# merbanan/rtl_433

Hardware: NVIDIA H100
Metric: IQ MS/s end-to-end demod+slice (higher is better)
Workload: dtype u8/int16/int32 fixed point

## Files before the change

### rtl_433_b200/csrc/r433b_api.cu

```cuda
#include <algorithm>
#include <cmath>
#include <cstdio>
#include <cstdlib>
#include <chrono>
#include <cstring>
#include <exception>
#include <atomic>
#include <mutex>
#include <string>
#include <thread>
#include <vector>

#include "../../include/r433b.h"
#include "../../include/r433b_abi.h"
#include "r433b_kernels.cuh"
#include "r433b_host.hpp"
#include "r433b_pulses.hpp"
#include "r433b_analyze.cuh"
#include "r433b_analyze_host.hpp"
#include "r433b_grab.cuh"

using namespace r433b;

#ifdef R433B_SIMT_EMU
// ... 32 lines not shown
    r433b_batch batch{};
    std::vector<uint64_t> offsets, lengths;
    bool processed = false, fetched = false;
    unsigned fpdm = 0;
    int enable_fm = 0;
    int n_sms = 132;
    int spoil_front = 0;
    size_t min_caps[3] = {0, 0, 0};
    Levels lv{};
    DevBuf d_data, d_offsets, d_train, d_pkgs, d_ppool, d_gpool, d_counters, d_am, d_fm;
    DevBuf d_devparams, d_lists, d_pairs, d_arena, d_cursor;
    size_t pkg_cap = 0, pool_cap = 0, arena_cap = 0;
    unsigned n_ook = 0, n_fsk = 0;
    unsigned n_pkgs = 0, pool_used = 0;
    unsigned long long event_bytes = 0, n_events = 0, n_samples = 0, n_gated = 0;
    HostBuf h_pkgs, h_ppool, h_gpool, h_pairs, h_events;
    r433b_timing timing{};
    cudaEvent_t ev[6]{};
    int pipeline_groups = 0;
    cudaStream_t s_in = nullptr, s_det = nullptr, s_out = nullptr;
    static constexpr int kMaxGroups = 16;
    cudaEvent_t ev_in[kMaxGroups]{}, ev_det[kMaxGroups]{}, ev_slc[kMaxGroups]{}, ev_t[4 * kMaxGroups]{}, ev_f[kMaxGroups]{}, ev_init = nullptr;
    DevBuf d_order;
    DevBuf d_ranges, d_state, d_lengths, d_stage, d_raw, d_log, d_amoff, d_chunks, d_tiles;
    std::vector<uint64_t> am_offsets;
    HostBuf h_ranges;
    bool d2h_done = false;
    bool pulse_mode = false;
    std::vector<PulseSet::Meta> pulse_meta;
    std::vector<uint32_t> dev_index;
    bool analyzed = false;
    std::vector<r433b_analysis> an;
    std::vector<r433b_guess> an_guess;
    std::vector<std::string> an_text;
    std::vector<r433b_pair> an_pairs;
    std::vector<uint8_t> an_events;
    DevBuf d_an, d_an_dev, d_an_gap, d_an_pairs, d_an_arena;
    std::thread worker;
    bool in_flight = false;
    int worker_rc = 0;
    r433b_batch sub_batch{};
    std::vector<uint64_t> sub_offsets, sub_lengths;
    r433b_results sub_res{};
    uint8_t const *grab_src = nullptr;
    unsigned grab_flip = 0;
    std::vector<uint32_t> p_events;
// ... 144 lines not shown
    if (char const *v = getenv("R433B_TEST_CAPS")) {
        unsigned long long c[3] = {0, 0, 0};
        sscanf(v, "%llu,%llu,%llu", &c[0], &c[1], &c[2]);
        for (int i = 0; i < 3; ++i) ctx->min_caps[i] = (size_t)c[i];
    }
    if (cudaDeviceGetAttribute(&ctx->n_sms, cudaDevAttrMultiProcessorCount, cuda_device) != cudaSuccess || ctx->n_sms <= 0)
        ctx->n_sms = 132;
    *out = ctx;
    return R433B_OK;
}

void r433b_destroy(r433b_ctx *ctx)
{
    if (!ctx) return;
    if (ctx->worker.joinable()) ctx->worker.join();
    cudaSetDevice(ctx->device);
    for (r433b_chain *ch : ctx->chains) {
        chain_free_device(ch);
        ch->ctx = nullptr;
    }
    for (DevBuf *b : {&ctx->d_data, &ctx->d_offsets, &ctx->d_train, &ctx->d_pkgs, &ctx->d_ppool, &ctx->d_gpool,
                 &ctx->d_counters, &ctx->d_am, &ctx->d_fm, &ctx->d_devparams, &ctx->d_lists, &ctx->d_pairs,
                 &ctx->d_arena, &ctx->d_cursor, &ctx->d_ranges, &ctx->d_state, &ctx->d_lengths, &ctx->d_stage, &ctx->d_raw, &ctx->d_log, &ctx->d_amoff, &ctx->d_chunks, &ctx->d_tiles,
                 &ctx->d_order, &ctx->d_an, &ctx->d_an_dev, &ctx->d_an_gap, &ctx->d_an_pairs, &ctx->d_an_arena,
                 &ctx->d_grab_prior, &ctx->d_grab_segs, &ctx->d_grab_stage})
        if (b->p) cudaFree(b->p);
    for (HostBuf *b : {&ctx->h_pkgs, &ctx->h_ppool, &ctx->h_gpool, &ctx->h_pairs, &ctx->h_events, &ctx->h_ranges})
        if (b->p) cudaFreeHost(b->p);
    for (auto &v : ctx->ev)
        if (v) cudaEventDestroy(v);
    for (auto *arr : {ctx->ev_in, ctx->ev_det, ctx->ev_slc})
        for (int i = 0; i < r433b_ctx::kMaxGroups; ++i)
            if (arr[i]) cudaEventDestroy(arr[i]);
    for (auto &v : ctx->ev_t)
        if (v) cudaEventDestroy(v);
    for (auto &v : ctx->ev_f)
        if (v) cudaEventDestroy(v);
    if (ctx->ev_init) cudaEventDestroy(ctx->ev_init);
    for (cudaStream_t st : {ctx->s_in, ctx->s_det, ctx->s_out})
        if (st) cudaStreamDestroy(st);
    delete ctx;
}

char const *r433b_last_error(r433b_ctx const *ctx) { return ctx ? ctx->err.c_str() : "no context"; }

int r433b_set_levels(r433b_ctx *ctx, int use_mag_est, float level_limit_db, float min_level_db, float min_snr_db)
{
// ... 65 lines not shown

int upload_slicer_tables(r433b_ctx *ctx, std::vector<uint32_t> const &rates, cudaStream_t st)
{
    size_t const n_devs = ctx->devs.size();
    std::vector<SlicerParams> sp(rates.size() * n_devs);
    for (size_t g = 0; g < rates.size(); ++g)
        for (size_t i = 0; i < n_devs; ++i) {
            sp[g * n_devs + i] = scale_device(ctx->devs[i], rates[g]);
            if (!ctx->gates.empty()) sp[g * n_devs + i].gate = ctx->gates[i].min_bits;
        }
    std::vector<unsigned> lists = slice_list(ctx->devs, 1), fsk = slice_list(ctx->devs, 2);
    ctx->n_ook = (unsigned)lists.size();
    ctx->n_fsk = (unsigned)fsk.size();
    lists.insert(lists.end(), fsk.begin(), fsk.end());
    if (int r = dev_reserve(ctx, ctx->d_devparams, std::max<size_t>(1, sp.size()) * sizeof(SlicerParams))) return r;
    if (int r = dev_reserve(ctx, ctx->d_lists, (lists.size() + 1) * sizeof(unsigned))) return r;
    size_t const stage_threads = (size_t)ctx->n_sms * kSliceCtasPerSm * kSliceThreads;
    if (int r = dev_reserve(ctx, ctx->d_stage, stage_threads * kStageWords * sizeof(uint32_t))) return r;
    if (!sp.empty()) CU(cudaMemcpyAsync(ctx->d_devparams.p, sp.data(), sp.size() * sizeof(SlicerParams), cudaMemcpyHostToDevice, st));
    if (!lists.empty()) CU(cudaMemcpyAsync(ctx->d_lists.p, lists.data(), lists.size() * sizeof(unsigned), cudaMemcpyHostToDevice, st));
    return R433B_OK;
}

void launch_slice(r433b_ctx *ctx, GroupRange *range, unsigned n_pkgs, unsigned rate_index, cudaStream_t st)
{
    unsigned const n_devs = (unsigned)ctx->devs.size();
    r433b_package *pkgs = (r433b_package *)ctx->d_pkgs.p;
    SliceParams q{};
    q.pkgs = pkgs;
    q.range = range;
    q.order = (unsigned const *)ctx->d_order.p;
    q.pulse_pool = (int const *)ctx->d_ppool.p;
    q.gap_pool = (int const *)ctx->d_gpool.p;
    q.dev = (SlicerParams const *)ctx->d_devparams.p + (size_t)rate_index * n_devs;
    q.n_devs = n_devs;
    q.ook_list = (unsigned const *)ctx->d_lists.p;
    q.fsk_list = q.ook_list + ctx->n_ook;
    q.n_ook = ctx->n_ook;
    q.n_fsk = ctx->n_fsk;
    q.pairs = (r433b_pair *)ctx->d_pairs.p;
    q.arena = (uint8_t *)ctx->d_arena.p;
    q.arena_cap = ctx->arena_cap;
    q.cursor = (unsigned long long *)ctx->d_cursor.p;
    q.stage = (uint32_t *)ctx->d_stage.p;
    unsigned const bgrid = (unsigned)ctx->n_sms * 2;
    R4_LAUNCH(k_bucket_count, bgrid, kBucketThreads, 0, st, range, pkgs, n_pkgs, n_devs);
    R4_LAUNCH(k_bucket_scan, 1, 1, 0, st, range);
    R4_LAUNCH(k_bucket_scatter, bgrid, kBucketThreads, 0, st, range, (r433b_package const *)pkgs, n_pkgs, (unsigned *)ctx->d_order.p);
    R4_LAUNCH(k_slice2, (unsigned)ctx->n_sms * kSliceCtasPerSm, kSliceThreads, 0, st, q);
}

int slice_ranges(r433b_ctx *ctx, std::vector<GroupRange> const &ranges, unsigned n_pkgs, cudaStream_t st)
{
    unsigned const n_devs = (unsigned)ctx->devs.size();
    unsigned long long cursor[4] = {0, 0, 0, 0};
    ctx->timing.slice_launches = 0;
    CU(cudaEventRecord(ctx->ev[2], st));
    if (n_pkgs && n_devs) {
        size_t const pair_bytes = (size_t)n_pkgs * n_devs * sizeof(r433b_pair);
        if (int r = dev_reserve(ctx, ctx->d_pairs, pair_bytes)) return r;
        if (int r = dev_reserve(ctx, ctx->d_order, (size_t)n_pkgs * sizeof(unsigned))) return r;
        if (int r = dev_reserve(ctx, ctx->d_ranges, ranges.size() * sizeof(GroupRange))) return r;
        if (int r = dev_reserve(ctx, ctx->d_cursor, 64)) return r;
        for (int attempt = 0; attempt < 3; ++attempt) {
            if (int r = dev_reserve(ctx, ctx->d_arena, ctx->arena_cap)) return r;
            CU(cudaMemsetAsync(ctx->d_pairs.p, 0, pair_bytes, st));
            CU(cudaMemsetAsync(ctx->d_cursor.p, 0, 64, st));
            CU(cudaMemcpyAsync(ctx->d_ranges.p, ranges.data(), ranges.size() * sizeof(GroupRange), cudaMemcpyHostToDevice, st));
            for (size_t g = 0; g < ranges.size(); ++g) {
                launch_slice(ctx, (GroupRange *)ctx->d_ranges.p + g, n_pkgs, (unsigned)g, st);
                CU(cudaGetLastError());
                ctx->timing.slice_launches++;
            }
            CU(cudaMemcpyAsync(cursor, ctx->d_cursor.p, sizeof(cursor), cudaMemcpyDeviceToHost, st));
            CU(cudaStreamSynchronize(st));
            if (!cursor[2]) break;
            ctx->arena_cap = (size_t)cursor[0] + (1u << 20);
            if (attempt == 2) return fail(ctx, R433B_EOVERFLOW, "event arena overflow");
        }
    }
    CU(cudaEventRecord(ctx->ev[3], st));
    CU(cudaEventSynchronize(ctx->ev[3]));
    cudaEventElapsedTime(&ctx->timing.slice_ms, ctx->ev[2], ctx->ev[3]);
    ctx->event_bytes = cursor[0];
// ... 235 lines not shown
        if (ctx->offsets[i + 1] - ctx->offsets[i] != stride) uniform = false;
    if (G == 0) {
        uint64_t const min_slice = SS == 4 ? (512u << 10) : (128u << 10);
        G = (total_bytes >= (256ull << 20) && stride >= (1u << 20)) ? (int)std::min<uint64_t>(r433b_ctx::kMaxGroups, stride / min_slice) : 1;
    }
    if (b->data_on_device && ctx->pipeline_groups == 0) G = 1;
    if (b->want_stages || !n_devs || !uniform || cf32) G = 1;
    uint64_t slice_samples = 0;
    if (G > 1) {
        uint64_t n_samp = stride / SS;
        uint64_t unit = (uint64_t)T;
        slice_samples = (n_samp / G + unit - 1) / unit * unit;
        if (slice_samples == 0 || slice_samples >= n_samp) G = 1;
        else G = (int)((n_samp + slice_samples - 1) / slice_samples);
        if (G > r433b_ctx::kMaxGroups) G = 1;
    }
    if (G > 1) {
        using clk = std::chrono::steady_clock;
        auto t_wall0 = clk::now();
        if (int r = dev_reserve(ctx, ctx->d_pkgs, ctx->pkg_cap * sizeof(r433b_package))) return r;
        if (int r = dev_reserve(ctx, ctx->d_order, ctx->pkg_cap * sizeof(unsigned))) return r;
        if (int r = dev_reserve(ctx, ctx->d_ppool, ctx->pool_cap * sizeof(int))) return r;
        if (int r = dev_reserve(ctx, ctx->d_gpool, ctx->pool_cap * sizeof(int))) return r;
        size_t const pair_cap_bytes = ctx->pkg_cap * n_devs * sizeof(r433b_pair);
        if (int r = dev_reserve(ctx, ctx->d_pairs, pair_cap_bytes)) return r;
        if (int r = dev_reserve(ctx, ctx->d_arena, ctx->arena_cap)) return r;
        if (int r = dev_reserve(ctx, ctx->d_ranges, G * sizeof(GroupRange))) return r;
        if (int r = dev_reserve(ctx, ctx->d_state, (size_t)b->n_streams * sizeof(StreamState))) return r;
        if (int r = host_reserve(ctx, ctx->h_ranges, G * sizeof(GroupRange))) return r;
        dp.pkgs = (r433b_package *)ctx->d_pkgs.p;
        dp.pkg_cap = (unsigned)std::min<size_t>(ctx->pkg_cap, 0xffffffffu);
        dp.pulse_pool = (int *)ctx->d_ppool.p;
        dp.gap_pool = (int *)ctx->d_gpool.p;
        dp.pool_cap = (unsigned)std::min<size_t>(ctx->pool_cap, 0xffffffffu);
        if (!ch) dp.state = (StreamState *)ctx->d_state.p;
        detect_ran = true;
        GroupRange *d_rg = (GroupRange *)ctx->d_ranges.p;
        GroupRange *h_rg = (GroupRange *)ctx->h_ranges.p;
        unsigned const *d_cnt = (unsigned const *)ctx->d_counters.p;
        unsigned long long const *d_cur = (unsigned long long const *)ctx->d_cursor.p;

        CU(cudaEventRecord(ctx->ev_init, 0));
        CU(cudaStreamWaitEvent(ctx->s_det, ctx->ev_init, 0));
        CU(cudaMemsetAsync(ctx->d_counters.p, 0, 64, ctx->s_det));
        CU(cudaMemsetAsync(ctx->d_cursor.p, 0, 64, ctx->s_det));
        CU(cudaMemsetAsync(ctx->d_pairs.p, 0, pair_cap_bytes, ctx->s_det));
// ... 127 lines not shown
        dp.pulse_pool = (int *)ctx->d_ppool.p;
        dp.gap_pool = (int *)ctx->d_gpool.p;
        dp.pool_cap = (unsigned)std::min<size_t>(ctx->pool_cap, 0xffffffffu);
        CU(cudaMemsetAsync(ctx->d_counters.p, 0, 64, st));
        if (b->n_streams) {
            launch_detect(dp, st, ctx->ev[4]);
            CU(cudaGetLastError());
            detect_launches++;
            detect_ran = true;
        }
        CU(cudaMemcpyAsync(counters, ctx->d_counters.p, sizeof(counters), cudaMemcpyDeviceToHost, st));
        CU(cudaStreamSynchronize(st));
        if (!counters[2]) break;
        ctx->pkg_cap = std::max<size_t>(ctx->pkg_cap, (size_t)counters[0] + 64);
        ctx->pool_cap = std::max<size_t>(ctx->pool_cap, (size_t)counters[1] + 4096);
        if (attempt == 2) return fail(ctx, R433B_EOVERFLOW, "package arena overflow");
    }
    if ((uint64_t)counters[0] * n_devs > 0xffffffffull)
        return fail(ctx, R433B_EOVERFLOW, "packages x devices exceeds the 32-bit pair index (r433b_package.first_pair)");
    ctx->n_pkgs = counters[0];
    ctx->pool_used = counters[1];
    GroupRange all{};
    all.pkg_end = ctx->n_pkgs;
    if (int r = slice_ranges(ctx, std::vector<GroupRange>{all}, ctx->n_pkgs, st)) return r;
    ctx->n_samples = used_bytes / SS;
    cudaEventElapsedTime(&ctx->timing.h2d_ms, ctx->ev[0], ctx->ev[1]);
    ctx->timing.front_ms = 0;
    if (detect_launches) {
        cudaEventElapsedTime(&ctx->timing.front_ms, ctx->ev[1], ctx->ev[4]);
        cudaEventElapsedTime(&ctx->timing.detect_ms, ctx->ev[4], ctx->ev[2]);
    } else
        cudaEventElapsedTime(&ctx->timing.detect_ms, ctx->ev[1], ctx->ev[2]);
    ctx->timing.front_launches = detect_launches;
    ctx->timing.front_redone = counters[4];
    ctx->timing.front_repairs = counters[5];
    ctx->timing.idle_skipped = counters[6];
    ctx->timing.idle_rewalks = counters[7];
    ctx->timing.chain_folds = counters[8];
    ctx->timing.chain_fm_rebuilds = counters[9];
    cudaEventElapsedTime(&ctx->timing.total_ms, ctx->ev[0], ctx->ev[3]);
    ctx->timing.d2h_ms = 0;
    ctx->timing.detect_launches = detect_launches;
    ctx->processed = true;
    finish_chain();
    return R433B_OK;
}

// ... 501 lines not shown
        ranges.back().pkg_end = j + 1;
    }
    for (uint32_t rate : rates)
        if (!rate) return fail(ctx, R433B_EINVAL, "a package has sample_rate 0");

    ctx->n_pkgs = n;
    ctx->pool_used = (unsigned)pp.size();
    ctx->n_samples = 0;
    ctx->event_bytes = ctx->n_events = ctx->n_gated = 0;
    ctx->timing = r433b_timing{};
    if (n) {
        if (int r = dev_reserve(ctx, ctx->d_pkgs, (size_t)n * sizeof(r433b_package))) return r;
        if (int r = dev_reserve(ctx, ctx->d_ppool, pp.size() * sizeof(int) + 16)) return r;
        if (int r = dev_reserve(ctx, ctx->d_gpool, gp.size() * sizeof(int) + 16)) return r;
        CU(cudaMemcpyAsync(ctx->d_pkgs.p, hp.data(), (size_t)n * sizeof(r433b_package), cudaMemcpyHostToDevice, st));
        CU(cudaMemcpyAsync(ctx->d_ppool.p, pp.data(), pp.size() * sizeof(int), cudaMemcpyHostToDevice, st));
        CU(cudaMemcpyAsync(ctx->d_gpool.p, gp.data(), gp.size() * sizeof(int), cudaMemcpyHostToDevice, st));
        CU(cudaStreamSynchronize(st));
    }
    if (n && n_devs) {
        size_t const arena_min = ctx->min_caps[2] ? ctx->min_caps[2] : (size_t)(1u << 20);
        if (ctx->arena_cap < arena_min) ctx->arena_cap = arena_min;
        if (int r = upload_slicer_tables(ctx, rates, st)) return r;
        if (int r = slice_ranges(ctx, ranges, n, st)) return r;
        ctx->timing.total_ms = ctx->timing.slice_ms;
    }
    ctx->processed = true;
    return R433B_OK;
}

}



namespace {

uint32_t package_rate(r433b_ctx const *ctx, r433b_package const &k)
{
    if (ctx->pulse_mode && k.end_pos < ctx->pulse_meta.size()) return ctx->pulse_meta[k.end_pos].rate;
    return ctx->batch.samp_rate;
}

}

extern "C" {

int r433b_analyze(r433b_ctx *ctx, r433b_results const *res)
// ... 389 lines not shown
```

### rtl_433_b200/csrc/r433b_kernels.cuh

```cuda
#pragma once
#include <cuda_runtime.h>
#include <stdint.h>

#include "../../include/r433b.h"
#include "r433b_core.cuh"
#include "r433b_slice.cuh"
#include "r433b_detect.cuh"

namespace r433b {


__global__ void k_cf32_to_cs16(float4 const *in, uint2 *out, size_t n4)
{
    for (size_t i = (size_t)blockIdx.x * blockDim.x + threadIdx.x; i < n4; i += (size_t)gridDim.x * blockDim.x) {
        float4 v = __ldcs(in + i);
        float f[4] = {v.x, v.y, v.z, v.w};
        int s[4];
#pragma unroll
        for (int k = 0; k < 4; ++k) {
            float t = __fmul_rn(f[k], 32767.0f);
            int q = (t >= -2147483648.0f && t < 2147483648.0f) ? __float2int_rz(t) : (int)0x80000000;
            q = q < -32767 ? -32767 : (q > 32767 ? 32767 : q);
            s[k] = q;
        }
        uint2 o;
        o.x = (uint32_t)(uint16_t)(int16_t)s[0] | ((uint32_t)(uint16_t)(int16_t)s[1] << 16);
        o.y = (uint32_t)(uint16_t)(int16_t)s[2] | ((uint32_t)(uint16_t)(int16_t)s[3] << 16);
        out[i] = o;
    }
}


constexpr int kLenBuckets = 4;
__host__ __device__ inline int len_bucket(unsigned num_pulses)
{
    return num_pulses < 64 ? 0 : num_pulses < 160 ? 1 : num_pulses < 400 ? 2 : 3;
}

struct GroupRange {
    unsigned pkg_begin, pkg_end;
    unsigned pool_begin, pool_end;
    unsigned long long arena_begin, arena_end;
    unsigned long long events_end, gated_end;
    unsigned overflow;
    unsigned next;
    unsigned seg_begin[2][kLenBuckets], seg_count[2][kLenBuckets], seg_fill[2][kLenBuckets];
    unsigned groups[2];
};

__global__ void k_mark(GroupRange *r, int which, unsigned const *counters, unsigned long long const *cursor)
{
    if (which == 0) {
        r->pkg_begin = counters[0];
        r->pool_begin = counters[1];
    } else if (which == 1) {
        r->pkg_end = counters[0];
        r->pool_end = counters[1];
        r->overflow = counters[2];
        r->next = 0;
        for (int i = 0; i < 2 * kLenBuckets; ++i) (&r->seg_count[0][0])[i] = 0;
    } else if (which == 2) {
        r->arena_begin = cursor[0];
    } else {
        r->arena_end = cursor[0];
        r->events_end = cursor[1];
        r->gated_end = cursor[3];
        r->overflow |= (unsigned)cursor[2] << 1;
    }
}


constexpr int kBucketThreads = 256;
__global__ void __launch_bounds__(kBucketThreads) k_bucket_count(GroupRange *r, r433b_package *pkgs, unsigned n_pkgs, unsigned n_devs)
{
    unsigned const b0 = r->pkg_begin, b1 = r->pkg_end < n_pkgs ? r->pkg_end : n_pkgs;
    for (unsigned pk = b0 + blockIdx.x * kBucketThreads + threadIdx.x; pk < b1; pk += gridDim.x * kBucketThreads) {
        r433b_package const k = pkgs[pk];
        pkgs[pk].first_pair = pk * n_devs;
        atomicAdd(&r->seg_count[k.type == 1 ? 0 : 1][len_bucket(k.num_pulses)], 1u);
    }
}

__global__ void k_bucket_scan(GroupRange *r)
{
    unsigned at = 0;
    for (int t = 0; t < 2; ++t) {
        unsigned g = 0;
        for (int b = 0; b < kLenBuckets; ++b) {
            r->seg_begin[t][b] = at;
            r->seg_fill[t][b] = 0;
            at += r->seg_count[t][b];
            g += (r->seg_count[t][b] + 31) / 32;
        }
        r->groups[t] = g;
    }
    r->next = 0;
}

__global__ void __launch_bounds__(kBucketThreads) k_bucket_scatter(GroupRange *r, r433b_package const *pkgs, unsigned n_pkgs, unsigned *order)
{
    unsigned const b0 = r->pkg_begin, b1 = r->pkg_end < n_pkgs ? r->pkg_end : n_pkgs;
    for (unsigned pk = b0 + blockIdx.x * kBucketThreads + threadIdx.x; pk < b1; pk += gridDim.x * kBucketThreads) {
        r433b_package const k = pkgs[pk];
        int const t = k.type == 1 ? 0 : 1, b = len_bucket(k.num_pulses);
        unsigned const pos = r->seg_begin[t][b] + atomicAdd(&r->seg_fill[t][b], 1u);
        order[b0 + pos] = pk;
    }
}

struct SliceParams {
    r433b_package const *pkgs;
    GroupRange *range;
    unsigned const *order;
    int const *pulse_pool, *gap_pool;
    SlicerParams const *dev;
    unsigned n_devs;
    unsigned const *ook_list, *fsk_list;
    unsigned n_ook, n_fsk;
    r433b_pair *pairs;
    uint8_t *arena;
    unsigned long long arena_cap;
    unsigned long long *cursor;
    uint32_t *stage;
};

constexpr int kSliceThreads = 128;
constexpr unsigned kStageWords = 1024;
constexpr int kSliceCtasPerSm = 8;

__shared__ uint32_t g_slice_win[kSliceWindow][kSliceThreads];
__shared__ unsigned g_slice_seg[2][kSliceThreads];
struct SliceWindow {
    static constexpr bool kOn = true;
    __device__ __forceinline__ static uint32_t &slot(unsigned s) { return g_slice_win[s][threadIdx.x]; }
};

__global__ void __launch_bounds__(kSliceThreads, kSliceCtasPerSm) k_slice2(SliceParams p)
{
    unsigned const lane = threadIdx.x & 31, warp = threadIdx.x >> 5;
    GroupRange const *rg = p.range;
    unsigned const pk_begin = rg->pkg_begin;
    unsigned const groups_ook = rg->groups[0], groups_fsk = rg->groups[1];
    unsigned const items_ook = p.n_ook * groups_ook, items = items_ook + p.n_fsk * groups_fsk;
    uint32_t *stage = p.stage + ((size_t)blockIdx.x * kSliceThreads + threadIdx.x) * kStageWords;
    for (;;) {
        unsigned item = 0;
        if (lane == 0) item = atomicAdd(&p.range->next, 1u);
        item = __shfl_sync(0xffffffffu, item, 0);
        if (item >= items) break;
        int const t = item < items_ook ? 0 : 1;
        unsigned const rel = t ? item - items_ook : item;
        unsigned const groups = t ? groups_fsk : groups_ook;
        unsigned const slot = rel / groups;
        unsigned g = rel - slot * groups;
        unsigned const dev = (t ? p.fsk_list : p.ook_list)[slot];
        int b = 0;
        for (; b < kLenBuckets - 1; ++b) {
            unsigned const gb = (rg->seg_count[t][b] + 31) / 32;
            if (g < gb) break;
            g -= gb;
        }
        unsigned const in_seg = g * 32 + lane;
        bool const active = in_seg < rg->seg_count[t][b];
        unsigned const pk = active ? p.order[pk_begin + rg->seg_begin[t][b] + in_seg] : 0;
        SlicerParams const sp = p.dev[dev];
        PulseView pv;
        pv.pulse = p.pulse_pool;
        pv.gap = p.gap_pool;
        pv.n = 0;
        if (active) {
            r433b_package const k = p.pkgs[pk];
            pv.pulse = p.pulse_pool + k.pulse_off;
            pv.gap = p.gap_pool + k.pulse_off;
            pv.n = k.num_pulses;
        }
        unsigned bytes = 0, nev = 0, ng1 = 0, ngN = 0, wb = 0;
        if (active) {
            EventWriterT<SliceWindow> w;
            w.init(stage, kStageWords, (unsigned)sp.gate);
            slice_dispatch(pv, sp, w);
            bytes = w.committed * 4;
            wb = w.wb;
            nev = w.events;
            ng1 = w.gated1;
            ngN = w.gatedN;
        }
        unsigned incl = bytes;
#pragma unroll
        for (int o = 1; o < 32; o <<= 1) {
            unsigned v = __shfl_up_sync(0xffffffffu, incl, o);
            if ((int)lane >= o) incl += v;
        }
        unsigned const total = __shfl_sync(0xffffffffu, incl, 31);
        unsigned evs = nev, dropped = ng1 + ngN;
#pragma unroll
        for (int o = 16; o > 0; o >>= 1) {
            evs += __shfl_xor_sync(0xffffffffu, evs, o);
            dropped += __shfl_xor_sync(0xffffffffu, dropped, o);
// ... 54 lines not shown
```

### rtl_433_b200/csrc/r433b_slice.cuh

```cuda
#pragma once
#include <stdint.h>
#include "r433b_core.cuh"

namespace r433b {

constexpr int kBbRows = 50;
constexpr int kBbCols = 128;

#ifdef __CUDA_ARCH__
R4_HD float fmul(float a, float b) { return __fmul_rn(a, b); }
R4_HD float fadd(float a, float b) { return __fadd_rn(a, b); }
R4_HD float fdiv(float a, float b) { return __fdiv_rn(a, b); }
R4_HD double dadd(double a, double b) { return __dadd_rn(a, b); }
R4_HD double dmul(double a, double b) { return __dmul_rn(a, b); }
#else
R4_HD float fmul(float a, float b) { volatile float r = a * b; return r; }
R4_HD float fadd(float a, float b) { volatile float r = a + b; return r; }
R4_HD float fdiv(float a, float b) { volatile float r = a / b; return r; }
R4_HD double dadd(double a, double b) { volatile double r = a + b; return r; }
R4_HD double dmul(double a, double b) { volatile double r = a * b; return r; }
#endif

struct SlicerParams {
    int modulation;
// ... 231 lines not shown
        } else if ((bits > max_bits ? bits : max_bits) < gate) {
            if (num_rows == 1) gated1++; else gatedN++;
            reset_event();
            return;
        } else if (one_word) {
            pos = ev_start + 1;
        } else {
            close_row();
            if (dirty) {
                put(pos, row_hw);
                pos += 1;
            }
        }
        put(ev_start, one_word ? 0xffu | (bits << 8) | (syncs << 13) | (bswap32(acc) << 16)
                               : num_rows | (dirty ? 0x80u : 0u) | (free_row << 8) | ((pos - ev_start) << 16));
        committed = pos;
        events++;
        reset_event();
    }
};
using EventWriter = EventWriterT<>;


struct PulseView {
    int const *pulse;
    int const *gap;
    unsigned n;
};

enum {
    kModOokMc = 3, kModOokPcm = 4, kModOokPpm = 5, kModOokPwm = 6, kModOokPiwmRaw = 8, kModOokDmc = 9,
    kModOokOsv1 = 10, kModOokPiwmDc = 11, kModOokNrzs = 12, kModOokRzi = 13,
    kModFskPcm = 16, kModFskPwm = 17, kModFskMc = 18
};

R4_HD bool device_takes(int modulation, int package_type)
{
    if (package_type == 1) return modulation >= 3 && modulation <= 13 && modulation != 7;
    return modulation >= 16 && modulation <= 18;
}

R4_HD int iabs(int v) { return v < 0 ? -v : v; }
R4_HD bool within(int v, int nominal, int tol) { return v >= nominal - tol && v <= nominal + tol; }
R4_HD int symbol_at(PulseView const &p, unsigned k) { return (k & 1) ? p.gap[k >> 1] : p.pulse[k >> 1]; }

enum { kRowNone = 0, kRowAdd, kRowSync, kRowClear, kRowIfOpen };
enum { kEmitNone = 0, kEmitAlways, kEmitIfRows, kEmitIfData, kEmitIfRow0, kEmitElseRowIfOpen };
struct Step {
    int ones;
    int zeros;
    int row;
    int bit;
    int emit;
    bool stop_if_emitted, clear_after;
    int post_zeros;
};

struct SlicerState {
    unsigned k, total;
    int b0, b1, b2, b3, b4, b5;
    float f_short, f_long;
    int i0, i1, i2;
    int since;
    double edge;
    bool pending;
    int cv, cg;
};

R4_HD void slicer_advance(PulseView const &p, SlicerState &st, unsigned k)
{
    st.k = k;
    if (k < st.total) {
        st.cv = p.pulse[k];
        st.cg = p.gap[k];
    }
}

constexpr int kModAny = -1;
template <int MOD>
R4_HD int slicer_family(SlicerParams const &t)
{
    if (MOD != kModAny) return MOD;
    int const m = t.modulation;
    return m == kModFskPwm ? (int)kModOokPwm : m == kModFskPcm ? (int)kModOokPcm : m == kModFskMc ? (int)kModOokMc : m;
}

template <int MOD>
R4_HD bool slicer_begin0(PulseView const &p, SlicerParams const &t, SlicerState &st)
{
    st.k = 0;
    st.cv = st.cg = 0;
    st.total = p.n;
    st.since = 0;
    st.pending = false;
    int const big = 0x7fffffff;
    switch (slicer_family<MOD>(t)) {
    case kModOokPwm: {
        if (!(t.ok & 1)) return false;
        st.b4 = st.b5 = 0;
        if (t.s_tol > 0) {
            st.b0 = t.s_short - t.s_tol; st.b1 = t.s_short + t.s_tol;
            st.b2 = t.s_long - t.s_tol;  st.b3 = t.s_long + t.s_tol;
            if (t.s_sync > 0) { st.b4 = t.s_sync - t.s_tol; st.b5 = t.s_sync + t.s_tol; }
        } else if (t.s_sync <= 0) {
            st.b0 = 0; st.b1 = (t.s_short + t.s_long) / 2 + 1;
            st.b2 = st.b1 - 1; st.b3 = big;
        } else if (t.s_sync < t.s_short) {
            st.b4 = 0; st.b5 = (t.s_sync + t.s_short) / 2 + 1;
            st.b0 = st.b5 - 1; st.b1 = (t.s_short + t.s_long) / 2 + 1;
            st.b2 = st.b1 - 1; st.b3 = big;
        } else if (t.s_sync < t.s_long) {
// ... 15 lines not shown
            st.b2 = t.s_long - t.s_tol;  st.b3 = t.s_long + t.s_tol;
            if (t.s_sync > 0) { st.b4 = t.s_sync - t.s_tol; st.b5 = t.s_sync + t.s_tol; }
        } else {
            st.b0 = 0;
            st.b1 = (t.s_short + t.s_long) / 2 + 1;
            st.b2 = st.b1 - 1;
            st.b3 = t.s_gap ? t.s_gap : t.s_reset;
        }
        return true;
    }
    case kModOokPcm: {
        if (!(t.ok & 1) || t.s_long == 0) return false;
        float f_short = t.f_short, f_long = t.f_long;
        int const gap_limit = t.s_gap ? t.s_gap : t.s_reset;
        int tol = t.s_tol;
        if (tol <= 0) tol = t.s_long / 4;
        bool const rz = t.s_short != t.s_long;
        int need = rz ? 4 : 12;
        int preamble = 0;
        unsigned const N = p.n;
        if (rz) {
            for (unsigned n = 0; n < N; ++n) {
                int sw = 0, lw = 0, cnt = 0;
                while (n < N && within(p.pulse[n], t.s_short, tol) && within(p.pulse[n] + p.gap[n], t.s_long, tol)) {
                    sw += p.pulse[n];
                    lw += p.pulse[n] + p.gap[n];
                    cnt++;
                    n++;
                }
                if (cnt >= need) {
                    f_long = fdiv((float)cnt, (float)lw);
                    f_short = fdiv((float)cnt, (float)sw);
                    need = cnt;
                    preamble = cnt;
                }
            }
            if (preamble == 0) {
                int sw = 0, lw = 0, cnt = 0;
                for (unsigned n = 0; n < N; ++n) {
                    if (within(p.pulse[n], t.s_short, tol) && within(p.pulse[n] + p.gap[n], t.s_long, tol)) {
                        sw += p.pulse[n];
                        lw += p.pulse[n] + p.gap[n];
                        cnt++;
                    }
                }
                if (cnt > 8) {
                    f_long = fdiv((float)cnt, (float)lw);
                    f_short = fdiv((float)cnt, (float)sw);
                }
            }
        } else {
            for (unsigned n = 0; n < N; ++n) {
                int wsum = 0, cnt = 0;
                while (n < N && (int)dadd((double)fmul((float)p.pulse[n], f_short), 0.5) == 1
                        && (int)dadd((double)fmul((float)p.gap[n], f_long), 0.5) == 1) {
                    wsum += p.pulse[n] + p.gap[n];
                    cnt += 2;
                    n++;
                }
                if (cnt >= need) {
                    f_short = f_long = fdiv((float)cnt, (float)wsum);
                    need = cnt;
                    preamble = cnt;
                }
            }
            if (preamble == 0) {
                int wsum = 0, cnt = 0;
                for (unsigned n = 0; n < N; ++n) {
                    if (within(p.pulse[n], t.s_short, tol)) { wsum += p.pulse[n]; cnt += 1; }
                    if (within(p.pulse[n], 2 * t.s_short, tol)) { wsum += p.pulse[n]; cnt += 2; }
                    if (within(p.gap[n], t.s_long, tol)) { wsum += p.gap[n]; cnt += 1; }
                    if (within(p.gap[n], 2 * t.s_long, tol)) { wsum += p.gap[n]; cnt += 2; }
                }
                if (cnt > 20) f_short = f_long = fdiv((float)cnt, (float)wsum);
            }
        }
        st.f_short = f_short;
        st.f_long = f_long;
        st.i0 = gap_limit;
        st.i1 = gap_limit / t.s_long;
        st.i2 = tol;
        return true;
    }
    case kModOokMc:
        if (!(t.ok & 1)) return false;
        st.edge = dmul((double)t.s_short, 1.5);
        st.i0 = t.s_short - t.s_tol;
        st.i1 = t.s_short * 2 + t.s_tol;
        st.pending = true;
        return true;
    case kModOokDmc: case kModOokPiwmRaw: case kModOokPiwmDc:
        if (!(t.ok & 1)) return false;
        st.total = p.n * 2;
        return true;
    case kModOokNrzs:
        return (t.ok & 1) && t.s_short != 0;
    case kModOokOsv1: {
        if (!(t.ok & 1)) return false;
        int const half_lo = t.s_short / 2, half_hi = t.s_short * 3 / 2, sync_lo = 2 * half_hi;
        int pre = 0;
        unsigned n;
        for (n = 0; n < p.n; ++n) {
            if (p.pulse[n] > half_lo && p.gap[n] > half_lo) {
                pre++;
                if (p.gap[n] > half_hi) break;
            } else {
                return false;
            }
        }
        if (pre != 12) return false;
        ++n;
        if (n >= (unsigned)kMaxPulses) return false;
        if (p.pulse[n] < sync_lo || p.gap[n] < sync_lo) return false;
        st.since = 0;
        if (p.gap[n] > p.pulse[n]) {
            st.since = 1;
            st.pending = true;
        }
        st.k = n + 1;
        st.i0 = half_hi;
        return true;
    }
    case kModOokRzi:
        if (!(t.ok & 2) || t.s_long == 0) return false;
        st.i0 = t.s_long - t.s_short;
        st.since = 1;
        return true;
    default:
        return false;
    }
}

template <int MOD>
R4_HD bool slicer_begin(PulseView const &p, SlicerParams const &t, SlicerState &st)
{
    if (!slicer_begin0<MOD>(p, t, st)) return false;
    slicer_advance(p, st, st.k);
    return true;
}

template <int MOD>
R4_HD Step slicer_step(PulseView const &p, SlicerParams const &t, SlicerState &st)
{
    Step s;
    s.ones = s.zeros = s.post_zeros = 0;
    s.row = kRowNone;
    s.bit = 0;
    s.emit = kEmitNone;
    s.stop_if_emitted = s.clear_after = false;
    unsigned const n = st.k;
    switch (slicer_family<MOD>(t)) {
    case kModOokPwm: {
        int v = st.cv, g = st.cg;
        if (v > st.b0 && v < st.b1) s.ones = 1;
        else if (v > st.b2 && v < st.b3) s.zeros = 1;
        else if (v > st.b4 && v < st.b5) s.row = kRowSync;
        else if (v <= st.b0) { }
        else s.row = kRowAdd;
        if (n == st.total - 1 || g > t.s_reset) s.emit = kEmitIfRows;
        else if (t.s_gap > 0 && g > t.s_gap) s.emit = kEmitElseRowIfOpen;
        slicer_advance(p, st, n + 1);
        break;
    }
    case kModOokPpm: {
        int g = st.cg;
// ... 164 lines not shown
        if (first) w.add_bits(s.ones ? 1 : 0, first);
        if (s.ones && s.zeros) w.add_bits(0, s.zeros);
    }
    if (s.row == kRowAdd || s.row == kRowSync) w.first_row();
    bool const open = w.num_rows > 0 && w.last_row_bits() > 0;
    bool const want_row = s.row == kRowAdd || (s.row == kRowSync && w.last_row_bits() > 0)
            || ((s.row == kRowIfOpen || s.emit == kEmitElseRowIfOpen) && open);
    if (want_row) w.add_row();
    if (s.row == kRowSync) w.syncs++;
    if (s.row == kRowClear) w.reset_event();
    if (s.bit) w.add_bits(s.bit - 1, 1);
    bool go = false;
    if (s.emit == kEmitAlways) go = true;
    else if (s.emit == kEmitIfRows) go = w.num_rows > 0;
    else if (s.emit == kEmitIfData) go = w.first_row_bits() > 0 || w.num_rows > 1;
    else if (s.emit == kEmitIfRow0) go = w.first_row_bits() > 0;
    if (go) w.emit();
    if (s.clear_after) w.reset_event();
    if (go && s.stop_if_emitted) return false;
    if (s.post_zeros) w.add_bits(0, s.post_zeros);
    return true;
}

template <int MOD, class W>
R4_HD void slice_loop(PulseView const &p, SlicerParams const &t, W &w)
{
    SlicerState st;
    if (!slicer_begin<MOD>(p, t, st)) return;
    while (st.k < st.total || st.pending) {
        Step s = slicer_step<MOD>(p, t, st);
        if (!slicer_apply(s, w)) break;
    }
}

template <class W>
R4_HD void slice_dispatch(PulseView const &p, SlicerParams const &t, W &w)
{
    switch (t.modulation) {
    case kModOokPwm: case kModFskPwm: slice_loop<kModOokPwm>(p, t, w); return;
    case kModOokPpm: slice_loop<kModOokPpm>(p, t, w); return;
    case kModOokPcm: case kModFskPcm: slice_loop<kModOokPcm>(p, t, w); return;
    case kModOokMc: case kModFskMc: slice_loop<kModOokMc>(p, t, w); return;
    default: break;
    }
    slice_loop<kModAny>(p, t, w);
}

}
```

Baseline: 132,000.

## Sort packages by exact length and transpose pulse data into coalesced per-warp copies

Replaces the four coarse length buckets with a per-length histogram sort (longest first), so each 32-lane slicing group holds packages of equal length. During scatter it also copies each group's pulse/gap pairs into a transposed interleaved buffer (stride 32), so lanes in a warp read adjacent 8-byte PulseGap entries instead of scattered reads from separate pulse and gap pools. This is meant to cut warp divergence and uncoalesced global loads in the slicer. The cost is an extra copy pass, a larger scratch buffer that can overflow and disable groups, and a single-warp scan kernel.

```diff
diff --git a/rtl_433_b200/csrc/r433b_api.cu b/rtl_433_b200/csrc/r433b_api.cu
--- a/rtl_433_b200/csrc/r433b_api.cu
+++ b/rtl_433_b200/csrc/r433b_api.cu
@@ -78,6 +78,7 @@
     static constexpr int kMaxGroups = 16;
     cudaEvent_t ev_in[kMaxGroups]{}, ev_det[kMaxGroups]{}, ev_slc[kMaxGroups]{}, ev_t[4 * kMaxGroups]{}, ev_f[kMaxGroups]{}, ev_init = nullptr;
     DevBuf d_order;
+    DevBuf d_sort, d_copy;
     DevBuf d_ranges, d_state, d_lengths, d_stage, d_raw, d_log, d_amoff, d_chunks, d_tiles;
     std::vector<uint64_t> am_offsets;
     HostBuf h_ranges;
@@ -268,7 +269,7 @@
     for (DevBuf *b : {&ctx->d_data, &ctx->d_offsets, &ctx->d_train, &ctx->d_pkgs, &ctx->d_ppool, &ctx->d_gpool,
                  &ctx->d_counters, &ctx->d_am, &ctx->d_fm, &ctx->d_devparams, &ctx->d_lists, &ctx->d_pairs,
                  &ctx->d_arena, &ctx->d_cursor, &ctx->d_ranges, &ctx->d_state, &ctx->d_lengths, &ctx->d_stage, &ctx->d_raw, &ctx->d_log, &ctx->d_amoff, &ctx->d_chunks, &ctx->d_tiles,
-                 &ctx->d_order, &ctx->d_an, &ctx->d_an_dev, &ctx->d_an_gap, &ctx->d_an_pairs, &ctx->d_an_arena,
+                 &ctx->d_order, &ctx->d_sort, &ctx->d_copy, &ctx->d_an, &ctx->d_an_dev, &ctx->d_an_gap, &ctx->d_an_pairs, &ctx->d_an_arena,
                  &ctx->d_grab_prior, &ctx->d_grab_segs, &ctx->d_grab_stage})
         if (b->p) cudaFree(b->p);
     for (HostBuf *b : {&ctx->h_pkgs, &ctx->h_ppool, &ctx->h_gpool, &ctx->h_pairs, &ctx->h_events, &ctx->h_ranges})
@@ -380,16 +381,30 @@
     return R433B_OK;
 }
 
+int reserve_sort(r433b_ctx *ctx, size_t pkgs, size_t pool_entries, cudaStream_t st)
+{
+    size_t const cap0 = ctx->d_sort.cap;
+    if (int r = dev_reserve(ctx, ctx->d_sort, (4 * kLenBins + pkgs / 32 + 3) * sizeof(unsigned))) return r;
+    if (ctx->d_sort.cap != cap0) CU(cudaMemsetAsync(ctx->d_sort.p, 0, 2 * kLenBins * sizeof(unsigned), st));
+    return dev_reserve(ctx, ctx->d_copy, (pool_entries + 2 * 32 * (size_t)kMaxPulses) * sizeof(PulseGap));
+}
+
 void launch_slice(r433b_ctx *ctx, GroupRange *range, unsigned n_pkgs, unsigned rate_index, cudaStream_t st)
 {
+    SortScratch ss;
+    ss.hist = (unsigned *)ctx->d_sort.p;
+    ss.fill = ss.hist + 2 * kLenBins;
+    ss.base = ss.fill + 2 * kLenBins;
+    ss.copy = (PulseGap *)ctx->d_copy.p;
+    ss.copy_cap = std::min<size_t>(ctx->d_copy.cap / sizeof(PulseGap), 0xffffffffu);
     unsigned const n_devs = (unsigned)ctx->devs.size();
     r433b_package *pkgs = (r433b_package *)ctx->d_pkgs.p;
     SliceParams q{};
     q.pkgs = pkgs;
     q.range = range;
     q.order = (unsigned const *)ctx->d_order.p;
-    q.pulse_pool = (int const *)ctx->d_ppool.p;
-    q.gap_pool = (int const *)ctx->d_gpool.p;
+    q.copy = ss.copy;
+    q.group_base = ss.base;
     q.dev = (SlicerParams const *)ctx->d_devparams.p + (size_t)rate_index * n_devs;
     q.n_devs = n_devs;
     q.ook_list = (unsigned const *)ctx->d_lists.p;
@@ -402,13 +417,14 @@
     q.cursor = (unsigned long long *)ctx->d_cursor.p;
     q.stage = (uint32_t *)ctx->d_stage.p;
     unsigned const bgrid = (unsigned)ctx->n_sms * 2;
-    R4_LAUNCH(k_bucket_count, bgrid, kBucketThreads, 0, st, range, pkgs, n_pkgs, n_devs);
-    R4_LAUNCH(k_bucket_scan, 1, 1, 0, st, range);
-    R4_LAUNCH(k_bucket_scatter, bgrid, kBucketThreads, 0, st, range, (r433b_package const *)pkgs, n_pkgs, (unsigned *)ctx->d_order.p);
+    R4_LAUNCH(k_bucket_count, bgrid, kBucketThreads, 0, st, range, pkgs, n_pkgs, n_devs, ss.hist);
+    R4_LAUNCH(k_bucket_scan, 1, 32, 0, st, range, ss);
+    R4_LAUNCH(k_bucket_scatter, bgrid, kBucketThreads, 0, st, range, (r433b_package const *)pkgs, n_pkgs, (unsigned *)ctx->d_order.p, ss,
+              (int const *)ctx->d_ppool.p, (int const *)ctx->d_gpool.p);
     R4_LAUNCH(k_slice2, (unsigned)ctx->n_sms * kSliceCtasPerSm, kSliceThreads, 0, st, q);
 }
 
-int slice_ranges(r433b_ctx *ctx, std::vector<GroupRange> const &ranges, unsigned n_pkgs, cudaStream_t st)
+int slice_ranges(r433b_ctx *ctx, std::vector<GroupRange> const &ranges, unsigned n_pkgs, size_t pool_entries, cudaStream_t st)
 {
     unsigned const n_devs = (unsigned)ctx->devs.size();
     unsigned long long cursor[4] = {0, 0, 0, 0};
@@ -418,6 +434,7 @@
         size_t const pair_bytes = (size_t)n_pkgs * n_devs * sizeof(r433b_pair);
         if (int r = dev_reserve(ctx, ctx->d_pairs, pair_bytes)) return r;
         if (int r = dev_reserve(ctx, ctx->d_order, (size_t)n_pkgs * sizeof(unsigned))) return r;
+        if (int r = reserve_sort(ctx, n_pkgs, pool_entries, st)) return r;
         if (int r = dev_reserve(ctx, ctx->d_ranges, ranges.size() * sizeof(GroupRange))) return r;
         if (int r = dev_reserve(ctx, ctx->d_cursor, 64)) return r;
         for (int attempt = 0; attempt < 3; ++attempt) {
@@ -699,6 +716,7 @@
         if (int r = dev_reserve(ctx, ctx->d_order, ctx->pkg_cap * sizeof(unsigned))) return r;
         if (int r = dev_reserve(ctx, ctx->d_ppool, ctx->pool_cap * sizeof(int))) return r;
         if (int r = dev_reserve(ctx, ctx->d_gpool, ctx->pool_cap * sizeof(int))) return r;
+        if (int r = reserve_sort(ctx, ctx->pkg_cap, ctx->pool_cap, ctx->s_det)) return r;
         size_t const pair_cap_bytes = ctx->pkg_cap * n_devs * sizeof(r433b_pair);
         if (int r = dev_reserve(ctx, ctx->d_pairs, pair_cap_bytes)) return r;
         if (int r = dev_reserve(ctx, ctx->d_arena, ctx->arena_cap)) return r;
@@ -872,7 +890,7 @@
     ctx->pool_used = counters[1];
     GroupRange all{};
     all.pkg_end = ctx->n_pkgs;
-    if (int r = slice_ranges(ctx, std::vector<GroupRange>{all}, ctx->n_pkgs, st)) return r;
+    if (int r = slice_ranges(ctx, std::vector<GroupRange>{all}, ctx->n_pkgs, ctx->pool_used, st)) return r;
     ctx->n_samples = used_bytes / SS;
     cudaEventElapsedTime(&ctx->timing.h2d_ms, ctx->ev[0], ctx->ev[1]);
     ctx->timing.front_ms = 0;
@@ -1420,7 +1438,7 @@
         size_t const arena_min = ctx->min_caps[2] ? ctx->min_caps[2] : (size_t)(1u << 20);
         if (ctx->arena_cap < arena_min) ctx->arena_cap = arena_min;
         if (int r = upload_slicer_tables(ctx, rates, st)) return r;
-        if (int r = slice_ranges(ctx, ranges, n, st)) return r;
+        if (int r = slice_ranges(ctx, ranges, n, pp.size(), st)) return r;
         ctx->timing.total_ms = ctx->timing.slice_ms;
     }
     ctx->processed = true;
diff --git a/rtl_433_b200/csrc/r433b_kernels.cuh b/rtl_433_b200/csrc/r433b_kernels.cuh
--- a/rtl_433_b200/csrc/r433b_kernels.cuh
+++ b/rtl_433_b200/csrc/r433b_kernels.cuh
@@ -30,12 +30,6 @@
     }
 }
 
-
-constexpr int kLenBuckets = 4;
-__host__ __device__ inline int len_bucket(unsigned num_pulses)
-{
-    return num_pulses < 64 ? 0 : num_pulses < 160 ? 1 : num_pulses < 400 ? 2 : 3;
-}
 
 struct GroupRange {
     unsigned pkg_begin, pkg_end;
@@ -44,8 +38,7 @@
     unsigned long long events_end, gated_end;
     unsigned overflow;
     unsigned next;
-    unsigned seg_begin[2][kLenBuckets], seg_count[2][kLenBuckets], seg_fill[2][kLenBuckets];
-    unsigned groups[2];
+    unsigned count[2], groups[2];
 };
 
 __global__ void k_mark(GroupRange *r, int which, unsigned const *counters, unsigned long long const *cursor)
@@ -58,7 +51,6 @@
         r->pool_end = counters[1];
         r->overflow = counters[2];
         r->next = 0;
-        for (int i = 0; i < 2 * kLenBuckets; ++i) (&r->seg_count[0][0])[i] = 0;
     } else if (which == 2) {
         r->arena_begin = cursor[0];
     } else {
@@ -69,42 +61,119 @@
     }
 }
 
+constexpr unsigned kLenBins = kMaxPulses + 1;
+
+__host__ __device__ inline unsigned len_bin(unsigned num_pulses) { return num_pulses < kLenBins ? num_pulses : kMaxPulses; }
+__host__ __device__ inline unsigned copy_rows(unsigned len) { return len < (unsigned)kMaxPulses ? len + 1 : kMaxPulses; }
+
+struct SortScratch {
+    unsigned *hist;
+    unsigned *fill;
+    unsigned *base;
+    PulseGap *copy;
+    unsigned long long copy_cap;
+};
 
 constexpr int kBucketThreads = 256;
-__global__ void __launch_bounds__(kBucketThreads) k_bucket_count(GroupRange *r, r433b_package *pkgs, unsigned n_pkgs, unsigned n_devs)
+__global__ void __launch_bounds__(kBucketThreads) k_bucket_count(GroupRange *r, r433b_package *pkgs, unsigned n_pkgs, unsigned n_devs, unsigned *hist)
 {
     unsigned const b0 = r->pkg_begin, b1 = r->pkg_end < n_pkgs ? r->pkg_end : n_pkgs;
     for (unsigned pk = b0 + blockIdx.x * kBucketThreads + threadIdx.x; pk < b1; pk += gridDim.x * kBucketThreads) {
         r433b_package const k = pkgs[pk];
         pkgs[pk].first_pair = pk * n_devs;
-        atomicAdd(&r->seg_count[k.type == 1 ? 0 : 1][len_bucket(k.num_pulses)], 1u);
-    }
-}
-
-__global__ void k_bucket_scan(GroupRange *r)
-{
-    unsigned at = 0;
-    for (int t = 0; t < 2; ++t) {
-        unsigned g = 0;
-        for (int b = 0; b < kLenBuckets; ++b) {
-            r->seg_begin[t][b] = at;
-            r->seg_fill[t][b] = 0;
-            at += r->seg_count[t][b];
-            g += (r->seg_count[t][b] + 31) / 32;
-        }
-        r->groups[t] = g;
-    }
-    r->next = 0;
-}
-
-__global__ void __launch_bounds__(kBucketThreads) k_bucket_scatter(GroupRange *r, r433b_package const *pkgs, unsigned n_pkgs, unsigned *order)
-{
+        atomicAdd(&hist[(k.type == 1 ? 0 : kLenBins) + len_bin(k.num_pulses)], 1u);
+    }
+}
+
+__global__ void __launch_bounds__(32) k_bucket_scan(GroupRange *r, SortScratch s)
+{
+    constexpr unsigned kBins = 2 * kLenBins, kPer = (kBins + 31) / 32;
+    __shared__ unsigned hist[kPer * 32];
+    unsigned const lane = threadIdx.x;
+    auto len = [](unsigned i) { return i < kLenBins ? kMaxPulses - i : kLenBins + kMaxPulses - i; };
+    for (unsigned i = lane; i < kPer * 32; i += 32) hist[i] = i < kBins ? s.hist[(i < kLenBins ? 0 : kLenBins) + len(i)] : 0;
+    __syncwarp();
+    unsigned n0 = 0, n1 = 0;
+    for (unsigned j = 0; j < kPer; ++j) {
+        unsigned const i = lane * kPer + j;
+        (i < kLenBins ? n0 : n1) += hist[i];
+    }
+    unsigned at = n0 + n1;
+#pragma unroll
+    for (int o = 1; o < 32; o <<= 1) {
+        unsigned const v = __shfl_up_sync(0xffffffffu, at, o);
+        if ((int)lane >= o) at += v;
+    }
+    at -= n0 + n1;
+#pragma unroll
+    for (int o = 16; o > 0; o >>= 1) {
+        n0 += __shfl_xor_sync(0xffffffffu, n0, o);
+        n1 += __shfl_xor_sync(0xffffffffu, n1, o);
+    }
+    unsigned const g0 = (n0 + 31) / 32, g1 = (n1 + 31) / 32;
+    unsigned long long e = 0;
+    for (unsigned j = 0, a = at; j < kPer; ++j) {
+        unsigned const i = lane * kPer + j, n = hist[i];
+        unsigned const q = a - (i < kLenBins ? 0 : n0);
+        e += (unsigned long long)((q + n + 31) / 32 - (q + 31) / 32) * 32 * copy_rows(len(i));
+        a += n;
+    }
+    unsigned long long incl = e;
+#pragma unroll
+    for (int o = 1; o < 32; o <<= 1) {
+        unsigned long long const v = __shfl_up_sync(0xffffffffu, incl, o);
+        if ((int)lane >= o) incl += v;
+    }
+    unsigned long long const total = __shfl_sync(0xffffffffu, incl, 31);
+    bool const fits = total <= s.copy_cap;
+    e = incl - e;
+    for (unsigned j = 0; j < kPer; ++j) {
+        unsigned const i = lane * kPer + j, n = hist[i];
+        if (i >= kBins) break;
+        unsigned const t = i < kLenBins ? 0 : 1, b = t * kLenBins + len(i), q = at - (t ? n0 : 0);
+        s.fill[b] = at;
+        if (n) s.hist[b] = 0;
+        unsigned const size = 32 * copy_rows(len(i));
+        for (unsigned g = (q + 31) / 32; g * 32 < q + n; ++g, e += size) s.base[(t ? g0 : 0) + g] = (unsigned)e;
+        at += n;
+    }
+    if (lane == 0) {
+        s.base[g0 + g1] = (unsigned)total;
+        r->count[0] = n0;
+        r->count[1] = n1;
+        r->groups[0] = fits ? g0 : 0;
+        r->groups[1] = fits ? g1 : 0;
+        if (!fits) r->overflow |= 4;
+        r->next = 0;
+    }
+}
+
+__global__ void __launch_bounds__(kBucketThreads) k_bucket_scatter(GroupRange *r, r433b_package const *pkgs, unsigned n_pkgs, unsigned *order,
+                                                                  SortScratch s, int const *pulse_pool, int const *gap_pool)
+{
+    unsigned const lane = threadIdx.x & 31;
     unsigned const b0 = r->pkg_begin, b1 = r->pkg_end < n_pkgs ? r->pkg_end : n_pkgs;
-    for (unsigned pk = b0 + blockIdx.x * kBucketThreads + threadIdx.x; pk < b1; pk += gridDim.x * kBucketThreads) {
-        r433b_package const k = pkgs[pk];
-        int const t = k.type == 1 ? 0 : 1, b = len_bucket(k.num_pulses);
-        unsigned const pos = r->seg_begin[t][b] + atomicAdd(&r->seg_fill[t][b], 1u);
-        order[b0 + pos] = pk;
+    unsigned const n0 = r->count[0], g0 = r->groups[0], g1 = r->groups[1];
+    for (unsigned w = b0 + blockIdx.x * kBucketThreads + threadIdx.x - lane; w < b1; w += gridDim.x * kBucketThreads) {
+        unsigned const pk = w + lane;
+        unsigned dst = 0, rows = 0, off = 0;
+        if (pk < b1) {
+            r433b_package const k = pkgs[pk];
+            unsigned const t = k.type == 1 ? 0 : 1, len = len_bin(k.num_pulses);
+            unsigned const pos = atomicAdd(&s.fill[t * kLenBins + len], 1u);
+            order[b0 + pos] = pk;
+            unsigned const q = pos - (t ? n0 : 0);
+            if (q / 32 < (t ? g1 : g0)) {
+                dst = s.base[(t ? g0 : 0) + q / 32] + q % 32;
+                rows = copy_rows(len);
+                off = k.pulse_off;
+            }
+        }
+        for (int l = 0; l < 32; ++l) {
+            unsigned const n = __shfl_sync(0xffffffffu, rows, l), d = __shfl_sync(0xffffffffu, dst, l);
+            unsigned const o = __shfl_sync(0xffffffffu, off, l);
+            for (unsigned k = lane; k < n; k += 32) s.copy[d + 32 * k] = PulseGap{pulse_pool[o + k], gap_pool[o + k]};
+        }
     }
 }
 
@@ -112,7 +181,8 @@
     r433b_package const *pkgs;
     GroupRange *range;
     unsigned const *order;
-    int const *pulse_pool, *gap_pool;
+    PulseGap const *copy;
+    unsigned const *group_base;
     SlicerParams const *dev;
     unsigned n_devs;
     unsigned const *ook_list, *fsk_list;
@@ -152,28 +222,15 @@
         unsigned const rel = t ? item - items_ook : item;
         unsigned const groups = t ? groups_fsk : groups_ook;
         unsigned const slot = rel / groups;
-        unsigned g = rel - slot * groups;
+        unsigned const g = rel - slot * groups;
         unsigned const dev = (t ? p.fsk_list : p.ook_list)[slot];
-        int b = 0;
-        for (; b < kLenBuckets - 1; ++b) {
-            unsigned const gb = (rg->seg_count[t][b] + 31) / 32;
-            if (g < gb) break;
-            g -= gb;
-        }
-        unsigned const in_seg = g * 32 + lane;
-        bool const active = in_seg < rg->seg_count[t][b];
-        unsigned const pk = active ? p.order[pk_begin + rg->seg_begin[t][b] + in_seg] : 0;
+        unsigned const in_type = g * 32 + lane;
+        bool const active = in_type < rg->count[t];
+        unsigned const pk = active ? p.order[pk_begin + (t ? rg->count[0] : 0) + in_type] : 0;
         SlicerParams const sp = p.dev[dev];
-        PulseView pv;
-        pv.pulse = p.pulse_pool;
-        pv.gap = p.gap_pool;
-        pv.n = 0;
-        if (active) {
-            r433b_package const k = p.pkgs[pk];
-            pv.pulse = p.pulse_pool + k.pulse_off;
-            pv.gap = p.gap_pool + k.pulse_off;
-            pv.n = k.num_pulses;
-        }
+        PulseViewT<32> pv;
+        pv.w = p.copy + p.group_base[(t ? groups_ook : 0) + g] + lane;
+        pv.n = active ? len_bin(p.pkgs[pk].num_pulses) : 0;
         unsigned bytes = 0, nev = 0, ng1 = 0, ngN = 0, wb = 0;
         if (active) {
             EventWriterT<SliceWindow> w;
diff --git a/rtl_433_b200/csrc/r433b_slice.cuh b/rtl_433_b200/csrc/r433b_slice.cuh
--- a/rtl_433_b200/csrc/r433b_slice.cuh
+++ b/rtl_433_b200/csrc/r433b_slice.cuh
@@ -277,11 +277,23 @@
 using EventWriter = EventWriterT<>;
 
 
-struct PulseView {
+struct alignas(8) PulseGap {
+    int pulse, gap;
+};
+template <unsigned S>
+struct PulseViewT {
+    PulseGap const *w;
+    unsigned n;
+    R4_HD PulseGap row(unsigned k) const { return w[k * S]; }
+};
+template <>
+struct PulseViewT<1> {
     int const *pulse;
     int const *gap;
     unsigned n;
+    R4_HD PulseGap row(unsigned k) const { return PulseGap{pulse[k], gap[k]}; }
 };
+using PulseView = PulseViewT<1>;
 
 enum {
     kModOokMc = 3, kModOokPcm = 4, kModOokPpm = 5, kModOokPwm = 6, kModOokPiwmRaw = 8, kModOokDmc = 9,
@@ -297,7 +309,12 @@
 
 R4_HD int iabs(int v) { return v < 0 ? -v : v; }
 R4_HD bool within(int v, int nominal, int tol) { return v >= nominal - tol && v <= nominal + tol; }
-R4_HD int symbol_at(PulseView const &p, unsigned k) { return (k & 1) ? p.gap[k >> 1] : p.pulse[k >> 1]; }
+template <class PV>
+R4_HD int symbol_at(PV const &p, unsigned k)
+{
+    PulseGap const r = p.row(k >> 1);
+    return (k & 1) ? r.gap : r.pulse;
+}
 
 enum { kRowNone = 0, kRowAdd, kRowSync, kRowClear, kRowIfOpen };
 enum { kEmitNone = 0, kEmitAlways, kEmitIfRows, kEmitIfData, kEmitIfRow0, kEmitElseRowIfOpen };
@@ -322,12 +339,14 @@
     int cv, cg;
 };
 
-R4_HD void slicer_advance(PulseView const &p, SlicerState &st, unsigned k)
+template <class PV>
+R4_HD void slicer_advance(PV const &p, SlicerState &st, unsigned k)
 {
     st.k = k;
     if (k < st.total) {
-        st.cv = p.pulse[k];
-        st.cg = p.gap[k];
+        PulseGap const r = p.row(k);
+        st.cv = r.pulse;
+        st.cg = r.gap;
     }
 }
 
@@ -340,8 +359,8 @@
     return m == kModFskPwm ? (int)kModOokPwm : m == kModFskPcm ? (int)kModOokPcm : m == kModFskMc ? (int)kModOokMc : m;
 }
 
-template <int MOD>
-R4_HD bool slicer_begin0(PulseView const &p, SlicerParams const &t, SlicerState &st)
+template <int MOD, class PV>
+R4_HD bool slicer_begin0(PV const &p, SlicerParams const &t, SlicerState &st)
 {
     st.k = 0;
     st.cv = st.cg = 0;
@@ -403,11 +422,12 @@
         if (rz) {
             for (unsigned n = 0; n < N; ++n) {
                 int sw = 0, lw = 0, cnt = 0;
-                while (n < N && within(p.pulse[n], t.s_short, tol) && within(p.pulse[n] + p.gap[n], t.s_long, tol)) {
-                    sw += p.pulse[n];
-                    lw += p.pulse[n] + p.gap[n];
+                for (; n < N; ++n) {
+                    PulseGap const r = p.row(n);
+                    if (!within(r.pulse, t.s_short, tol) || !within(r.pulse + r.gap, t.s_long, tol)) break;
+                    sw += r.pulse;
+                    lw += r.pulse + r.gap;
                     cnt++;
-                    n++;
                 }
                 if (cnt >= need) {
                     f_long = fdiv((float)cnt, (float)lw);
@@ -419,9 +439,10 @@
             if (preamble == 0) {
                 int sw = 0, lw = 0, cnt = 0;
                 for (unsigned n = 0; n < N; ++n) {
-                    if (within(p.pulse[n], t.s_short, tol) && within(p.pulse[n] + p.gap[n], t.s_long, tol)) {
-                        sw += p.pulse[n];
-                        lw += p.pulse[n] + p.gap[n];
+                    PulseGap const r = p.row(n);
+                    if (within(r.pulse, t.s_short, tol) && within(r.pulse + r.gap, t.s_long, tol)) {
+                        sw += r.pulse;
+                        lw += r.pulse + r.gap;
                         cnt++;
                     }
                 }
@@ -433,11 +454,13 @@
         } else {
             for (unsigned n = 0; n < N; ++n) {
                 int wsum = 0, cnt = 0;
-                while (n < N && (int)dadd((double)fmul((float)p.pulse[n], f_short), 0.5) == 1
-                        && (int)dadd((double)fmul((float)p.gap[n], f_long), 0.5) == 1) {
-                    wsum += p.pulse[n] + p.gap[n];
+                for (; n < N; ++n) {
+                    PulseGap const r = p.row(n);
+                    if ((int)dadd((double)fmul((float)r.pulse, f_short), 0.5) != 1
+                            || (int)dadd((double)fmul((float)r.gap, f_long), 0.5) != 1)
+                        break;
+                    wsum += r.pulse + r.gap;
                     cnt += 2;
-                    n++;
                 }
                 if (cnt >= need) {
                     f_short = f_long = fdiv((float)cnt, (float)wsum);
@@ -448,10 +471,11 @@
             if (preamble == 0) {
                 int wsum = 0, cnt = 0;
                 for (unsigned n = 0; n < N; ++n) {
-                    if (within(p.pulse[n], t.s_short, tol)) { wsum += p.pulse[n]; cnt += 1; }
-                    if (within(p.pulse[n], 2 * t.s_short, tol)) { wsum += p.pulse[n]; cnt += 2; }
-                    if (within(p.gap[n], t.s_long, tol)) { wsum += p.gap[n]; cnt += 1; }
-                    if (within(p.gap[n], 2 * t.s_long, tol)) { wsum += p.gap[n]; cnt += 2; }
+                    PulseGap const r = p.row(n);
+                    if (within(r.pulse, t.s_short, tol)) { wsum += r.pulse; cnt += 1; }
+                    if (within(r.pulse, 2 * t.s_short, tol)) { wsum += r.pulse; cnt += 2; }
+                    if (within(r.gap, t.s_long, tol)) { wsum += r.gap; cnt += 1; }
+                    if (within(r.gap, 2 * t.s_long, tol)) { wsum += r.gap; cnt += 2; }
                 }
                 if (cnt > 20) f_short = f_long = fdiv((float)cnt, (float)wsum);
             }
@@ -482,9 +506,10 @@
         int pre = 0;
         unsigned n;
         for (n = 0; n < p.n; ++n) {
-            if (p.pulse[n] > half_lo && p.gap[n] > half_lo) {
+            PulseGap const r = p.row(n);
+            if (r.pulse > half_lo && r.gap > half_lo) {
                 pre++;
-                if (p.gap[n] > half_hi) break;
+                if (r.gap > half_hi) break;
             } else {
                 return false;
             }
@@ -492,9 +517,10 @@
         if (pre != 12) return false;
         ++n;
         if (n >= (unsigned)kMaxPulses) return false;
-        if (p.pulse[n] < sync_lo || p.gap[n] < sync_lo) return false;
+        PulseGap const sync = p.row(n);
+        if (sync.pulse < sync_lo || sync.gap < sync_lo) return false;
         st.since = 0;
-        if (p.gap[n] > p.pulse[n]) {
+        if (sync.gap > sync.pulse) {
             st.since = 1;
             st.pending = true;
         }
@@ -512,16 +538,16 @@
     }
 }
 
-template <int MOD>
-R4_HD bool slicer_begin(PulseView const &p, SlicerParams const &t, SlicerState &st)
+template <int MOD, class PV>
+R4_HD bool slicer_begin(PV const &p, SlicerParams const &t, SlicerState &st)
 {
     if (!slicer_begin0<MOD>(p, t, st)) return false;
     slicer_advance(p, st, st.k);
     return true;
 }
 
-template <int MOD>
-R4_HD Step slicer_step(PulseView const &p, SlicerParams const &t, SlicerState &st)
+template <int MOD, class PV>
+R4_HD Step slicer_step(PV const &p, SlicerParams const &t, SlicerState &st)
 {
     Step s;
     s.ones = s.zeros = s.post_zeros = 0;
@@ -732,8 +758,8 @@
     return true;
 }
 
-template <int MOD, class W>
-R4_HD void slice_loop(PulseView const &p, SlicerParams const &t, W &w)
+template <int MOD, class PV, class W>
+R4_HD void slice_loop(PV const &p, SlicerParams const &t, W &w)
 {
     SlicerState st;
     if (!slicer_begin<MOD>(p, t, st)) return;
@@ -743,8 +769,8 @@
     }
 }
 
-template <class W>
-R4_HD void slice_dispatch(PulseView const &p, SlicerParams const &t, W &w)
+template <class PV, class W>
+R4_HD void slice_dispatch(PV const &p, SlicerParams const &t, W &w)
 {
     switch (t.modulation) {
     case kModOokPwm: case kModFskPwm: slice_loop<kModOokPwm>(p, t, w); return;
```

New measurement: 142,400 (median of 6 runs). 1.08x the previous value.
